# Orbis-Tertius/tiny-ram-halo2

Measured on AMD Instinct MI355X. Metric: Pallas MSM pairs/s @ 2^24 + Fp NTT elems/s @ 2^22; 1/2/4/8 MI355X, higher is better.
Workload: dtype u255 (255-bit modular integers as 9 x 29/30-bit limbs in i32 / i64 lanes)

## Files before the change

tiny-ram-halo2_amd/csrc/msm.hip:

```cpp
#include <stdlib.h>
#include <string.h>

#include "ctx.h"
#include "devmem.h"
#include "curve_q4.h"
#include "hostcombine.h"
#include "hosthelper.h"
#include "hostplan.h"

namespace trh {

namespace {

using hostplan::MAX_C; using hostplan::MAX_C_FIXED; using hostplan::MSM_TILE; using hostplan::SMALL_C; using hostplan::SMALL_MAX_N;
using hostplan::PART_TILE; using hostplan::BIN_THREADS; using hostplan::BIN_PER_MAX; using hostplan::BIN_CAP_MAX; using hostplan::RANGE_BLOCK;
using hostplan::HEAVY_PIECES; using hostplan::SP_LISTS; using hostplan::SP_CNT; using hostplan::SP_PAD; using hostplan::SP_PARTS; using hostplan::SP_MAX_CHUNK;
using hostplan::num_windows;
static_assert(sizeof(XYZZMem) == hostplan::XYZZ_BYTES && sizeof(XYZZzMem) == hostplan::RAW_POINT_BYTES, "point sizes of the plan's scratch layout");
constexpr u32 SIGN_BIT = 0x80000000u;

constexpr int RECODE_THREADS_MAX = 1024;
template <class SF, int C, bool ONE_ROW , bool USE_LDS,
          bool FLAGS >
__global__ void __launch_bounds__(RECODE_THREADS_MAX) msm_recode_kernel(const uint4* __restrict__ scalars, size_t n, int mont, int c_arg, int W,
                                                         u32* __restrict__ digits, u32* __restrict__ bin_counts, int k2, u32 nbins, size_t sstride,
                                                         const uint4* __restrict__ tails ,
                                                         unsigned char* __restrict__ tile_flags, u32 tile_log, u32 tiles) {
    const size_t z = blockIdx.z;
    const u32 rows = ONE_ROW ? 1u : (u32)W;
    scalars += z * sstride * 2; digits += z * (size_t)W * n; bin_counts += z * (size_t)rows * nbins;
    extern __shared__ u32 lhist[];
    const u32 total = rows * nbins;
    if (USE_LDS) {
        for (u32 k = threadIdx.x; k < total; k += blockDim.x) lhist[k] = 0;
        __syncthreads();
    }
    const int c = C ? C : c_arg;
    const u32 mask = (1u << c) - 1u, half = 1u << (c - 1);
    const size_t stride = (size_t)gridDim.x * blockDim.x;
    size_t i = (size_t)blockIdx.x * blockDim.x + threadIdx.x;
    uint4 lo = make_uint4(0, 0, 0, 0), hi = lo;
    if (i < n) {
        const uint4* src = (tails && i == n - 1) ? tails + 2 * z : scalars + 2 * i;
        lo = src[0]; hi = src[1];
        asm volatile("" : "+v"(lo.x), "+v"(lo.y), "+v"(lo.z), "+v"(lo.w), "+v"(hi.x), "+v"(hi.y), "+v"(hi.z), "+v"(hi.w));
    }
    while (i < n) {
        u32 w[8] = {lo.x, lo.y, lo.z, lo.w, hi.x, hi.y, hi.z, hi.w};
        {
            const size_t nx = i + stride < n ? i + stride : i;
            const uint4* src = (tails && nx == n - 1) ? tails + 2 * z : scalars + 2 * nx;
            lo = src[0]; hi = src[1];
        }
        if (mont) fe_store(fe_from_mont(fe_load<SF>(w)), w);
        u32 carry = 0;
        u32* dg = digits + i;
        u32 row = 0;
        size_t slot = i;
        auto emit = [&](u32 raw) {
            raw += carry;
            u32 bucket, sign = 0;
            if (raw > half) { bucket = (1u << c) - raw; carry = 1; sign = SIGN_BIT; }
            else { bucket = raw; carry = 0; }
            *dg = bucket ? (bucket | sign) : 0u;
            if (FLAGS) {
                const unsigned long long nz = __ballot(bucket != 0);
                const u32 lane = threadIdx.x & 63u;
                if (bucket && ((nz & ((1ull << lane) - 1ull)) == 0ull || (slot & (((size_t)1 << tile_log) - 1)) < 64))
                    tile_flags[z * tiles + (slot >> tile_log)] = 1;
                slot += n;
            }
            if (bucket) {
                const u32 bin = (bucket - 1u) >> k2;
                if (USE_LDS) atomicAdd(&lhist[row + bin], 1u);
                else atomicAdd(&bin_counts[(size_t)row + bin], 1u);
            }
            dg += n;
            if (!ONE_ROW) row += nbins;
        };
        if constexpr (C != 0) {
            constexpr int WC = 255 / C + 1;
#pragma unroll
            for (int j = 0; j < WC; ++j) {
                const int b = j * C, k = b >> 5, s = b & 31;
                const u32 a0 = k < 8 ? w[k < 8 ? k : 7] : 0u, a1 = (s + C > 32 && k + 1 < 8) ? w[k + 1 < 8 ? k + 1 : 7] : 0u;
                emit((s ? (a0 >> s) | (a1 << ((32 - s) & 31)) : a0) & mask);
            }
        } else {
            for (int j = 0; j < W; ++j) {
                const u32 raw = w[0] & mask;
#pragma unroll
                for (int k = 0; k < 7; ++k) w[k] = (w[k] >> c) | (w[k + 1] << (32 - c));
                w[7] >>= c;
                emit(raw);
            }
        }
        i += stride;
    }
    if (USE_LDS) {
        __syncthreads();
        for (u32 k = threadIdx.x; k < total; k += blockDim.x) {
            const u32 v = lhist[k];
            if (v) atomicAdd(&bin_counts[k], v);
        }
    }
}

struct ZeroRanges { uint4* p[4]; u32 n16[4]; };
__global__ void __launch_bounds__(256) msm_zero_ranges_kernel(const ZeroRanges z) {
    const uint4 zero = make_uint4(0, 0, 0, 0);
#pragma unroll
    for (int k = 0; k < 4; ++k)
        for (u32 i = blockIdx.x * blockDim.x + threadIdx.x; i < z.n16[k]; i += gridDim.x * blockDim.x) z.p[k][i] = zero;
}

__global__ void __launch_bounds__(1024) msm_offsets_kernel(u32* __restrict__ counts, u32* __restrict__ starts, u32 nb1, u32* __restrict__ oversize, u32 bin_cap,
                                                           u32* __restrict__ totals ) {
    const size_t z = blockIdx.z;
    counts += z * (size_t)gridDim.x * nb1; starts += z * (size_t)gridDim.x * nb1;
    __shared__ u32 part[1024];
    const int j = blockIdx.x, t = threadIdx.x;
    u32* cnt = counts + (size_t)j * nb1;
    u32* st = starts + (size_t)j * nb1;
    const u32 per = (nb1 + 1023u) / 1024u;
    const u32 lo = t * per < nb1 ? t * per : nb1, hi = (lo + per < nb1) ? lo + per : nb1;
    u32 sum = 0, biggest = 0;
    for (u32 b = lo; b < hi; ++b) { const u32 v = cnt[b]; sum += v; biggest = v > biggest ? v : biggest; }
    if (oversize && biggest > bin_cap) atomicMax(oversize + z * gridDim.x + blockIdx.x, biggest);
    part[t] = sum;
    __syncthreads();
    for (int off = 1; off < 1024; off <<= 1) {
        u32 v = (t >= off) ? part[t - off] : 0;
        __syncthreads();
        part[t] += v;
        __syncthreads();
    }
    if (totals && t == 1023) totals[z * gridDim.x + blockIdx.x] = part[1023];
    u32 run = part[t] - sum;
    for (u32 b = lo; b < hi; ++b) {
        u32 cv = cnt[b];
        st[b] = run;
        cnt[b] = run;
        run += cv;
    }
}

constexpr int PART_THREADS = 1024;
__global__ void __launch_bounds__(PART_THREADS) msm_partition_kernel(const u32* __restrict__ digits, u32* __restrict__ bin_cursor,
                                                                     u32* __restrict__ parted, size_t n, int k2, u32 nbins, int idx_bits,
                                                                     const unsigned char* __restrict__ tile_flags ) {
    const size_t z = blockIdx.z;
    if (tile_flags && !tile_flags[z * gridDim.x + blockIdx.x]) return;
    digits += z * (size_t)gridDim.y * n; parted += z * (size_t)gridDim.y * n; bin_cursor += z * (size_t)gridDim.y * nbins;
    extern __shared__ u32 lds[];
    u32* stage = lds;
    u32* cnt = lds + PART_TILE;
    u32* lbase = cnt + nbins;
    u32* gbase = lbase + nbins;
    __shared__ u32 scan[PART_THREADS];
    const int j = blockIdx.y;
    const size_t t0 = (size_t)blockIdx.x * PART_TILE;
    const size_t t1 = t0 + PART_TILE < n ? t0 + PART_TILE : n;
    const u32* dg = digits + (size_t)j * n;
    for (u32 k = threadIdx.x; k < nbins; k += blockDim.x) cnt[k] = 0;
    __syncthreads();
    constexpr int PER = PART_TILE / PART_THREADS;
    u32 mine[PER];
#pragma unroll
    for (int q = 0; q < PER; ++q) {
        const size_t i = t0 + threadIdx.x + (size_t)q * PART_THREADS;
        mine[q] = i < t1 ? dg[i] : 0u;
    }
#pragma unroll
    for (int q = 0; q < PER; ++q) {
        const u32 b = mine[q] & ~SIGN_BIT;
        if (b) atomicAdd(&cnt[(b - 1u) >> k2], 1u);
    }
    __syncthreads();
    {
        const u32 per = (nbins + PART_THREADS - 1) / PART_THREADS;
        const u32 lo = threadIdx.x * per < nbins ? threadIdx.x * per : nbins, hi = lo + per < nbins ? lo + per : nbins;
        u32 sum = 0;
        for (u32 k = lo; k < hi; ++k) sum += cnt[k];
        scan[threadIdx.x] = sum;
        __syncthreads();
        for (int off = 1; off < PART_THREADS; off <<= 1) {
            const u32 v = ((int)threadIdx.x >= off) ? scan[threadIdx.x - off] : 0;
            __syncthreads();
            scan[threadIdx.x] += v;
            __syncthreads();
        }
        u32 run = scan[threadIdx.x] - sum;
        for (u32 k = lo; k < hi; ++k) {
            const u32 v = cnt[k];
            lbase[k] = run;
            gbase[k] = v ? atomicAdd(&bin_cursor[(size_t)j * nbins + k], v) : 0u;
            run += v;
        }
    }
    __syncthreads();
    for (u32 k = threadIdx.x; k < nbins; k += blockDim.x) cnt[k] = 0;
    __syncthreads();
    const u32 low_mask = (1u << k2) - 1u;
#pragma unroll
    for (int q = 0; q < PER; ++q) {
        const u32 e = mine[q];
        const u32 b = e & ~SIGN_BIT;
        if (b) {
            const u32 bm = b - 1u, bin = bm >> k2;
            const u32 r = atomicAdd(&cnt[bin], 1u);
            stage[lbase[bin] + r] = (u32)(t0 + threadIdx.x + (size_t)q * PART_THREADS) | ((bm & low_mask) << idx_bits) | (e & SIGN_BIT);
        }
    }
    __syncthreads();
    u32* out = parted + (size_t)j * n;
    const u32 wave = threadIdx.x >> 6, lane = threadIdx.x & 63u;
    for (u32 bin = wave; bin < nbins; bin += PART_THREADS / 64) {
        const u32 c = cnt[bin], lb = lbase[bin], gb = gbase[bin];
        for (u32 k = lane; k < c; k += 64) out[gb + k] = stage[lb + k];
    }
}

constexpr int BS_CHUNK = 8192;
constexpr int BS_THREADS = 512;

__device__ __forceinline__ u32 bin_of_position(const u32* __restrict__ bin_ends, u32 nbins, u32 pos) {
    u32 lo = 0, hi = nbins;
    while (lo < hi) {
        const u32 mid = (lo + hi) >> 1;
        if (bin_ends[mid] > pos) hi = mid; else lo = mid + 1;
    }
    return lo;
}

template <bool SCATTER>
__global__ void __launch_bounds__(BS_THREADS) msm_bucket_pass_kernel(const u32* __restrict__ parted, const u32* __restrict__ bin_starts,
                                                                     const u32* __restrict__ bin_ends, u32* __restrict__ bucket_cnt ,
                                                                     u32* __restrict__ sorted, size_t n, int k2, u32 nbins, int idx_bits, u32 nbk,
                                                                     const u32* __restrict__ oversize) {
    const size_t z = blockIdx.z;
    {
        const size_t Wz = gridDim.y;
        parted += z * Wz * n; sorted += z * Wz * n; bin_starts += z * Wz * nbins; bin_ends += z * Wz * nbins;
        bucket_cnt += z * Wz * (nbk + 1);
    }
    if (oversize && oversize[z * gridDim.y + blockIdx.y] == 0u) return;
    __shared__ u32 cnt[128], tbase[128], gbase[128];
    __shared__ u32 stage[SCATTER ? BS_CHUNK : 1];
    const int j = blockIdx.y;
    const u32* bs = bin_starts + (size_t)j * nbins;
    const u32* be = bin_ends + (size_t)j * nbins;
    const u32 total = be[nbins - 1];
    const u32 c0 = blockIdx.x * BS_CHUNK;
    if (c0 >= total) return;
    const u32 c1 = c0 + BS_CHUNK < total ? c0 + BS_CHUNK : total;
    const u32 nsub = 1u << k2, low_mask = nsub - 1u, idx_mask = (1u << idx_bits) - 1u;
    const u32* src = parted + (size_t)j * n;
    u32* dst = sorted + (size_t)j * n;
    u32* bc = bucket_cnt + (size_t)j * (nbk + 1);
    const u32 wave = threadIdx.x >> 6, lane = threadIdx.x & 63u;
    for (u32 bin = bin_of_position(be, nbins, c0); bin < nbins; ++bin) {
        const u32 lo = bs[bin] > c0 ? bs[bin] : c0;
        if (lo >= c1) break;
        const u32 hi = be[bin] < c1 ? be[bin] : c1;
        if (hi <= lo) continue;
        if (hi - lo <= 64u) {
            if (threadIdx.x < hi - lo) {
                const u32 e = src[lo + threadIdx.x];
                u32* cell = &bc[(bin << k2) + ((e >> idx_bits) & low_mask) + 1u];
                if (!SCATTER) atomicAdd(cell, 1u);
                else dst[atomicAdd(cell, 1u)] = (e & idx_mask) | (e & SIGN_BIT);
            }
            continue;
        }
        if (threadIdx.x < 128) cnt[threadIdx.x] = 0;
        __syncthreads();
        for (u32 i = lo + threadIdx.x; i < hi; i += blockDim.x) atomicAdd(&cnt[(src[i] >> idx_bits) & low_mask], 1u);
        __syncthreads();
        if (!SCATTER) {
            if (threadIdx.x < nsub && cnt[threadIdx.x]) atomicAdd(&bc[(bin << k2) + threadIdx.x + 1u], cnt[threadIdx.x]);
        } else {
            if (threadIdx.x == 0) {
                u32 r = 0;
                for (u32 k = 0; k < nsub; ++k) { tbase[k] = r; r += cnt[k]; }
            }
            if (threadIdx.x < nsub) {
                const u32 v = cnt[threadIdx.x];
                gbase[threadIdx.x] = v ? atomicAdd(&bc[(bin << k2) + threadIdx.x + 1u], v) : 0u;
            }
            __syncthreads();
            if (threadIdx.x < 128) cnt[threadIdx.x] = 0;
            __syncthreads();
            for (u32 i = lo + threadIdx.x; i < hi; i += blockDim.x) {
                const u32 e = src[i];
                const u32 sub = (e >> idx_bits) & low_mask;
                const u32 r = atomicAdd(&cnt[sub], 1u);
                stage[tbase[sub] + r] = (e & idx_mask) | (e & SIGN_BIT);
            }
            __syncthreads();
            for (u32 sub = wave; sub < nsub; sub += BS_THREADS / 64) {
                const u32 c = cnt[sub], sb = tbase[sub], gb = gbase[sub];
                for (u32 k = lane; k < c; k += 64) dst[gb + k] = stage[sb + k];
            }
        }
        __syncthreads();
    }
}

template <int PER>
__global__ void __launch_bounds__(BIN_THREADS) msm_bin_sort_kernel(const u32* __restrict__ parted, const u32* __restrict__ bin_starts, const u32* __restrict__ bin_ends,
                                                                   u32* __restrict__ sorted, u32* __restrict__ starts, u32* __restrict__ ends, size_t n, int k2, u32 nbins,
                                                                   int idx_bits, u32 nbk, const u32* __restrict__ oversize) {
    if (oversize[(size_t)blockIdx.z * gridDim.y + blockIdx.y] != 0u) return;
    extern __shared__ u32 bstage[];
    __shared__ u32 cnt[128], tbase[128], wave0_total;
    const size_t z = blockIdx.z, Wz = gridDim.y;
    const int j = blockIdx.y;
    const u32 bin = blockIdx.x;
    const size_t wrow = z * Wz + j;
    const u32 lo = bin_starts[wrow * nbins + bin], hi = bin_ends[wrow * nbins + bin];
    const u32 count = hi - lo;
    const u32 nsub = 1u << k2, low_mask = nsub - 1u, idx_mask = (1u << idx_bits) - 1u;
    const u32* src = parted + wrow * n + lo;
    u32* dst = sorted + wrow * n + lo;
    const u32 lane = threadIdx.x & 63u;
    if (threadIdx.x < 128) cnt[threadIdx.x] = 0;
    __syncthreads();
    u32 mine[PER];
#pragma unroll
    for (int q = 0; q < PER; ++q) {
        const u32 i = threadIdx.x + (u32)q * BIN_THREADS;
        mine[q] = (u32)q * BIN_THREADS < count ? src[i < count ? i : 0u] : 0u;
    }
#pragma unroll
    for (int q = 0; q < PER; ++q)
        if (threadIdx.x + (u32)q * BIN_THREADS < count) atomicAdd(&cnt[(mine[q] >> idx_bits) & low_mask], 1u);
    __syncthreads();
    u32 v = 0, x = 0;
    if (threadIdx.x < 128) {
        v = threadIdx.x < nsub ? cnt[threadIdx.x] : 0u;
        x = v;
#pragma unroll
        for (int off = 1; off < 64; off <<= 1) {
            const u32 y = __shfl_up(x, off, 64);
            if ((int)lane >= off) x += y;
        }
        if (threadIdx.x == 63) wave0_total = x;
    }
    __syncthreads();
    if (threadIdx.x < 128) {
        const u32 excl = x - v + (threadIdx.x >= 64 ? wave0_total : 0u);
        tbase[threadIdx.x] = excl;
        cnt[threadIdx.x] = 0;
        if (threadIdx.x < nsub) {
            const size_t b = wrow * (nbk + 1) + ((size_t)bin << k2) + threadIdx.x + 1u;
            starts[b] = lo + excl;
            ends[b] = lo + excl + v;
        }
        if (bin == 0 && threadIdx.x == 0) { starts[wrow * (nbk + 1)] = 0; ends[wrow * (nbk + 1)] = 0; }
    }
    __syncthreads();
#pragma unroll
    for (int q = 0; q < PER; ++q) {
        if (threadIdx.x + (u32)q * BIN_THREADS < count) {
            const u32 e = mine[q];
            const u32 sub = (e >> idx_bits) & low_mask;
            const u32 r = atomicAdd(&cnt[sub], 1u);
            bstage[tbase[sub] + r] = (e & idx_mask) | (e & SIGN_BIT);
        }
    }
    __syncthreads();
#pragma unroll
    for (int q = 0; q < PER; ++q) {
        const u32 i = threadIdx.x + (u32)q * BIN_THREADS;
        if (i < count) mine[q] = bstage[i];
    }
#pragma unroll
    for (int q = 0; q < PER; ++q) {
        const u32 i = threadIdx.x + (u32)q * BIN_THREADS;
        if (i < count) dst[i] = mine[q];
    }
}

__global__ void __launch_bounds__(RANGE_BLOCK) msm_bucket_block_sums_kernel(const u32* __restrict__ bucket_cnt, u32* __restrict__ block_sums, u32 nbk,
                                                                            const u32* __restrict__ oversize) {
    if (oversize && oversize[(size_t)blockIdx.z * gridDim.y + blockIdx.y] == 0u) return;
    __shared__ u32 part[RANGE_BLOCK / 64];
    const size_t z = blockIdx.z, Wz = gridDim.y;
    const u32 nb1 = nbk + 1, b = blockIdx.x * RANGE_BLOCK + threadIdx.x;
    u32 v = b < nb1 ? bucket_cnt[(z * Wz + blockIdx.y) * nb1 + b] : 0u;
#pragma unroll
    for (int off = 32; off > 0; off >>= 1) v += __shfl_down(v, off, 64);
    if ((threadIdx.x & 63) == 0) part[threadIdx.x >> 6] = v;
    __syncthreads();
    if (threadIdx.x == 0) {
        u32 t = 0;
        for (int k = 0; k < RANGE_BLOCK / 64; ++k) t += part[k];
        block_sums[(z * Wz + blockIdx.y) * gridDim.x + blockIdx.x] = t;
    }
}
__global__ void __launch_bounds__(RANGE_BLOCK) msm_bucket_ranges_kernel(u32* __restrict__ bucket_cnt, const u32* __restrict__ block_sums, u32* __restrict__ starts,
                                                                        u32* __restrict__ ends, u32 nbk, const u32* __restrict__ oversize) {
    if (oversize && oversize[(size_t)blockIdx.z * gridDim.y + blockIdx.y] == 0u) return;
    __shared__ u32 part[RANGE_BLOCK];
    __shared__ u32 before;
    const size_t z = blockIdx.z, Wz = gridDim.y;
    const int t = threadIdx.x;
    const u32 nb1 = nbk + 1, b = blockIdx.x * RANGE_BLOCK + t;
    const size_t row = (z * Wz + blockIdx.y) * nb1;
    const u32 c = b < nb1 ? bucket_cnt[row + b] : 0u;
    {
        u32 v = (u32)t < blockIdx.x ? block_sums[(z * Wz + blockIdx.y) * gridDim.x + t] : 0u;
        part[t] = v;
        __syncthreads();
        for (int s = RANGE_BLOCK / 2; s > 0; s >>= 1) {
            if (t < s) part[t] += part[t + s];
            __syncthreads();
        }
        if (t == 0) before = part[0];
        __syncthreads();
    }
    part[t] = c;
    __syncthreads();
    for (int off = 1; off < RANGE_BLOCK; off <<= 1) {
        const u32 v = (t >= off) ? part[t - off] : 0;
        __syncthreads();
        part[t] += v;
        __syncthreads();
    }
    if (b < nb1) {
        const u32 E = before + part[t], S = E - c;
        starts[row + b] = S; ends[row + b] = E; bucket_cnt[row + b] = S;
    }
}

template <class BF>
__device__ __forceinline__ void store_zrec(uint4* q, const Fy<BF>& x, const Fy<BF>& y) {
    q[0] = make_uint4((u32)x.l[0], (u32)x.l[1], (u32)x.l[2], (u32)x.l[3]); q[1] = make_uint4((u32)x.l[4], (u32)x.l[5], (u32)x.l[6], (u32)x.l[7]);
    q[2] = make_uint4((u32)y.l[0], (u32)y.l[1], (u32)y.l[2], (u32)y.l[3]); q[3] = make_uint4((u32)y.l[4], (u32)y.l[5], (u32)y.l[6], (u32)y.l[7]);
    q[4] = make_uint4((u32)-y.l[0], (u32)-y.l[1], (u32)-y.l[2], (u32)-y.l[3]); q[5] = make_uint4((u32)-y.l[4], (u32)-y.l[5], (u32)-y.l[6], (u32)-y.l[7]);
    q[6] = make_uint4((u32)x.l[8], (u32)y.l[8], (u32)-y.l[8], 0u);
    q[7] = make_uint4(0u, 0u, 0u, 0u);
}
template <class BF>
__global__ void __launch_bounds__(256) msm_convert_bases_kernel(const uint4* __restrict__ in, uint4* __restrict__ out, size_t n) {
    size_t i = (size_t)blockIdx.x * blockDim.x + threadIdx.x;
    if (i >= n) return;
    const uint4* p = in + i * 4;
    uint4 a = p[0], b = p[1], c = p[2], d = p[3];
    store_zrec(out + i * (ZREC / 16), fy_from_fe(fe_load<BF>(a.x, a.y, a.z, a.w, b.x, b.y, b.z, b.w)), fy_from_fe(fe_load<BF>(c.x, c.y, c.z, c.w, d.x, d.y, d.z, d.w)));
}

template <class BF>
__global__ void __launch_bounds__(256) msm_accumulate_seg_kernel(const uint4* __restrict__ bases_z, const u32* __restrict__ sorted,
                                                                 const u32* __restrict__ ends,
                                                                 XYZZzMem* __restrict__ first, XYZZzMem* __restrict__ last,
                                                                 XYZZzMem* __restrict__ direct, size_t n, u32 nbk, u32 nseg, u32 seg_len,
                                                                 const u32* __restrict__ lean_gate ) {
    const size_t z = blockIdx.z;
    if (lean_gate && lean_gate[z * gridDim.y + blockIdx.y] != 0u) return;
    {
        const size_t Wz = gridDim.y;
        sorted += z * Wz * n; ends += z * Wz * (nbk + 1);
        first += z * Wz * nseg; last += z * Wz * nseg; direct += z * Wz * (nbk + 1);
    }
    const u32 t = blockIdx.x * blockDim.x + threadIdx.x;
    const int j = blockIdx.y;
    if (t >= nseg) return;
    const u32 nb1 = nbk + 1;
    const u32* en = ends + (size_t)j * nb1;
    const u32 total = en[nbk];
    u32 pos = t * seg_len;
    if (pos >= total) return;
    const u32 stop = pos + seg_len < total ? pos + seg_len : total;
    u32 B;
    {
        u32 lo = 0, hi = nbk;
        while (lo < hi) {
            const u32 mid = (lo + hi) >> 1;
            if (en[mid] > pos) hi = mid; else lo = mid + 1;
        }
        B = lo;
    }
    u32 cur_end = en[B];
    const u32* lst = sorted + (size_t)j * n;
    XYZZzMem* my_first = first + (size_t)j * nseg + t;
    XYZZz<BF> acc = xyzzz_identity<BF>();
    bool is_first = true;
    bool fresh = true;
    struct Slot { u32 e; uint4 a, b, c, d, t; };
    auto issue = [&](Slot& sl, u32 entry) {
        sl.e = entry;
        const uint4* bp = bases_z + (size_t)(entry & ~SIGN_BIT) * (ZREC / 16);
        const uint4* yp = bp + 2 + ((entry >> 31) << 1);
        sl.a = bp[0]; sl.b = bp[1]; sl.c = yp[0]; sl.d = yp[1]; sl.t = bp[6];
    };
    auto unpack = [&](const Slot& sl, AffineZ<BF>& p) {
        p.x.l[0] = (i32)sl.a.x; p.x.l[1] = (i32)sl.a.y; p.x.l[2] = (i32)sl.a.z; p.x.l[3] = (i32)sl.a.w;
        p.x.l[4] = (i32)sl.b.x; p.x.l[5] = (i32)sl.b.y; p.x.l[6] = (i32)sl.b.z; p.x.l[7] = (i32)sl.b.w; p.x.l[8] = (i32)sl.t.x;
        p.y.l[0] = (i32)sl.c.x; p.y.l[1] = (i32)sl.c.y; p.y.l[2] = (i32)sl.c.z; p.y.l[3] = (i32)sl.c.w;
        p.y.l[4] = (i32)sl.d.x; p.y.l[5] = (i32)sl.d.y; p.y.l[6] = (i32)sl.d.z; p.y.l[7] = (i32)sl.d.w; p.y.l[8] = (i32)((sl.e >> 31) ? sl.t.z : sl.t.y);
    };
    const u32 last_pos = stop - 1;
    auto clamp = [&](u32 q) { return q < last_pos ? q : last_pos; };
    Slot s0, s1;
    issue(s0, lst[pos]);
    issue(s1, lst[clamp(pos + 1)]);
    u32 e_ahead = lst[clamp(pos + 2)];
    auto step = [&](Slot& sl) {
        if (pos == cur_end) {
            store_raw(is_first ? my_first : direct + (size_t)j * nb1 + B, acc);
            is_first = false;
            fresh = true;
            int walked = 0;
            do { ++B; cur_end = en[B]; } while (cur_end <= pos && ++walked < 4);
            if (cur_end <= pos) {
                u32 lo = B + 1, hi = nbk;
                while (lo < hi) {
                    const u32 mid = (lo + hi) >> 1;
                    if (en[mid] > pos) hi = mid; else lo = mid + 1;
                }
                B = lo;
// ... 1309 lines not shown
```

Baseline: 1.048 billion.

## Flatten partition write-out and swizzle blocks across XCDs

The partition kernel now remaps its block ids so consecutive work items land on the same XCD (8-way swizzle). The final copy from LDS stage to global output no longer walks bins per wave. Each thread instead takes a flat stage slot, finds its bin from a compact staged word, and writes to the slot position plus a per-bin delta (global base minus local base). This is meant to fix load imbalance from small or uneven bins and to improve L2 locality, at the cost of an extra LDS lookup per element and re-encoding the output word.

Result: no change. 1.055 billion, median of 6 (+0.6%).

```diff
diff --git a/tiny-ram-halo2_amd/csrc/msm.hip b/tiny-ram-halo2_amd/csrc/msm.hip
--- a/tiny-ram-halo2_amd/csrc/msm.hip
+++ b/tiny-ram-halo2_amd/csrc/msm.hip
@@ -146,20 +146,31 @@
 }
 
 constexpr int PART_THREADS = 1024;
+constexpr int PART_LOCAL_BITS = 14;
+constexpr u32 PART_XCDS = 8;
+static_assert(PART_TILE == 1 << PART_LOCAL_BITS, "the staged word keeps the index inside the tile in PART_LOCAL_BITS bits");
+static_assert(PART_LOCAL_BITS + (MAX_C - 1) <= 31 && PART_LOCAL_BITS + (MAX_C_FIXED - 1) <= 31, "staged word: tile index, bucket - 1 < 2^(c - 1), sign");
 __global__ void __launch_bounds__(PART_THREADS) msm_partition_kernel(const u32* __restrict__ digits, u32* __restrict__ bin_cursor,
                                                                      u32* __restrict__ parted, size_t n, int k2, u32 nbins, int idx_bits,
                                                                      const unsigned char* __restrict__ tile_flags ) {
     const size_t z = blockIdx.z;
-    if (tile_flags && !tile_flags[z * gridDim.x + blockIdx.x]) return;
+    u32 tile = blockIdx.x, j = blockIdx.y;
+    {
+        const u32 items = gridDim.x * gridDim.y, per = items / PART_XCDS, id = blockIdx.x + gridDim.x * blockIdx.y;
+        if (id < per * PART_XCDS) {
+            const u32 m = (id % PART_XCDS) * per + id / PART_XCDS;
+            tile = m % gridDim.x; j = m / gridDim.x;
+        }
+    }
+    if (tile_flags && !tile_flags[z * gridDim.x + tile]) return;
     digits += z * (size_t)gridDim.y * n; parted += z * (size_t)gridDim.y * n; bin_cursor += z * (size_t)gridDim.y * nbins;
     extern __shared__ u32 lds[];
     u32* stage = lds;
     u32* cnt = lds + PART_TILE;
     u32* lbase = cnt + nbins;
-    u32* gbase = lbase + nbins;
+    u32* delta = lbase + nbins;
     __shared__ u32 scan[PART_THREADS];
-    const int j = blockIdx.y;
-    const size_t t0 = (size_t)blockIdx.x * PART_TILE;
+    const size_t t0 = (size_t)tile * PART_TILE;
     const size_t t1 = t0 + PART_TILE < n ? t0 + PART_TILE : n;
     const u32* dg = digits + (size_t)j * n;
     for (u32 k = threadIdx.x; k < nbins; k += blockDim.x) cnt[k] = 0;
@@ -193,15 +204,15 @@
         u32 run = scan[threadIdx.x] - sum;
         for (u32 k = lo; k < hi; ++k) {
             const u32 v = cnt[k];
+            const u32 gb = v ? atomicAdd(&bin_cursor[(size_t)j * nbins + k], v) : 0u;
             lbase[k] = run;
-            gbase[k] = v ? atomicAdd(&bin_cursor[(size_t)j * nbins + k], v) : 0u;
+            delta[k] = gb - run;
             run += v;
         }
     }
     __syncthreads();
     for (u32 k = threadIdx.x; k < nbins; k += blockDim.x) cnt[k] = 0;
     __syncthreads();
-    const u32 low_mask = (1u << k2) - 1u;
 #pragma unroll
     for (int q = 0; q < PER; ++q) {
         const u32 e = mine[q];
@@ -209,15 +220,28 @@
         if (b) {
             const u32 bm = b - 1u, bin = bm >> k2;
             const u32 r = atomicAdd(&cnt[bin], 1u);
-            stage[lbase[bin] + r] = (u32)(t0 + threadIdx.x + (size_t)q * PART_THREADS) | ((bm & low_mask) << idx_bits) | (e & SIGN_BIT);
+            stage[lbase[bin] + r] = (threadIdx.x + (u32)q * PART_THREADS) | (bm << PART_LOCAL_BITS) | (e & SIGN_BIT);
         }
     }
     __syncthreads();
     u32* out = parted + (size_t)j * n;
-    const u32 wave = threadIdx.x >> 6, lane = threadIdx.x & 63u;
-    for (u32 bin = wave; bin < nbins; bin += PART_THREADS / 64) {
-        const u32 c = cnt[bin], lb = lbase[bin], gb = gbase[bin];
-        for (u32 k = lane; k < c; k += 64) out[gb + k] = stage[lb + k];
+    const u32 total = scan[PART_THREADS - 1], low_mask = (1u << k2) - 1u, local_mask = (1u << PART_LOCAL_BITS) - 1u;
+#pragma unroll
+    for (int q = 0; q < PER; ++q) {
+        const u32 p = threadIdx.x + (u32)q * PART_THREADS;
+        mine[q] = stage[p < total ? p : 0u];
+    }
+    u32 dst[PER];
+#pragma unroll
+    for (int q = 0; q < PER; ++q) {
+        const u32 p = threadIdx.x + (u32)q * PART_THREADS;
+        dst[q] = delta[p < total ? (mine[q] & ~SIGN_BIT) >> (PART_LOCAL_BITS + k2) : 0u] + p;
+    }
+#pragma unroll
+    for (int q = 0; q < PER; ++q) {
+        const u32 p = threadIdx.x + (u32)q * PART_THREADS;
+        const u32 w = mine[q];
+        if (p < total) out[dst[q]] = ((u32)t0 + (w & local_mask)) | (((w >> PART_LOCAL_BITS) & low_mask) << idx_bits) | (w & SIGN_BIT);
     }
 }
 
```

## Reuse counting-pass ranks and flatten scatter in MSM partition kernel

Applied to the files above, without the earlier changes.

The partition kernel now records each element's rank from the first LDS atomic counting pass, packing two 16-bit ranks per register. This removes the second counter reset and the second round of LDS atomics. The staged word holds the full bucket-minus-one and the tile-local index. The final write-out becomes one flat loop over all staged slots that decodes the bin with bitfield extracts and adds a per-bin global delta, replacing the per-wave-per-bin loop that left lanes idle on small bins. The cost is more live registers, per-slot decode work and a new bit-budget constraint checked by a static_assert.

Result: no change. 1.067 billion before, 1.067 billion after (median of 2 runs) (-0.0%).

```diff
diff --git a/tiny-ram-halo2_amd/csrc/msm.hip b/tiny-ram-halo2_amd/csrc/msm.hip
--- a/tiny-ram-halo2_amd/csrc/msm.hip
+++ b/tiny-ram-halo2_amd/csrc/msm.hip
@@ -146,6 +146,8 @@
 }
 
 constexpr int PART_THREADS = 1024;
+constexpr int PART_TILE_LOG = 14;
+static_assert(PART_TILE == 1 << PART_TILE_LOG && hostplan::MAX_C - 1 + PART_TILE_LOG + 1 <= 32 && hostplan::MAX_C_FIXED <= hostplan::MAX_C, "staged word of msm_partition_kernel");
 __global__ void __launch_bounds__(PART_THREADS) msm_partition_kernel(const u32* __restrict__ digits, u32* __restrict__ bin_cursor,
                                                                      u32* __restrict__ parted, size_t n, int k2, u32 nbins, int idx_bits,
                                                                      const unsigned char* __restrict__ tile_flags ) {
@@ -156,7 +158,7 @@
     u32* stage = lds;
     u32* cnt = lds + PART_TILE;
     u32* lbase = cnt + nbins;
-    u32* gbase = lbase + nbins;
+    u32* gdelta = lbase + nbins;
     __shared__ u32 scan[PART_THREADS];
     const int j = blockIdx.y;
     const size_t t0 = (size_t)blockIdx.x * PART_TILE;
@@ -171,10 +173,15 @@
         const size_t i = t0 + threadIdx.x + (size_t)q * PART_THREADS;
         mine[q] = i < t1 ? dg[i] : 0u;
     }
+    u32 rank2[PER / 2];
 #pragma unroll
     for (int q = 0; q < PER; ++q) {
         const u32 b = mine[q] & ~SIGN_BIT;
-        if (b) atomicAdd(&cnt[(b - 1u) >> k2], 1u);
+        if (!(q & 1)) rank2[q / 2] = 0u;
+        if (b) {
+            const u32 r = atomicAdd(&cnt[(b - 1u) >> k2], 1u);
+            rank2[q / 2] = (q & 1) ? (r << 16) | rank2[q / 2] : r;
+        }
     }
     __syncthreads();
     {
@@ -194,30 +201,29 @@
         for (u32 k = lo; k < hi; ++k) {
             const u32 v = cnt[k];
             lbase[k] = run;
-            gbase[k] = v ? atomicAdd(&bin_cursor[(size_t)j * nbins + k], v) : 0u;
+            gdelta[k] = (v ? atomicAdd(&bin_cursor[(size_t)j * nbins + k], v) : 0u) - run;
             run += v;
         }
     }
     __syncthreads();
-    for (u32 k = threadIdx.x; k < nbins; k += blockDim.x) cnt[k] = 0;
-    __syncthreads();
-    const u32 low_mask = (1u << k2) - 1u;
 #pragma unroll
     for (int q = 0; q < PER; ++q) {
         const u32 e = mine[q];
         const u32 b = e & ~SIGN_BIT;
         if (b) {
-            const u32 bm = b - 1u, bin = bm >> k2;
-            const u32 r = atomicAdd(&cnt[bin], 1u);
-            stage[lbase[bin] + r] = (u32)(t0 + threadIdx.x + (size_t)q * PART_THREADS) | ((bm & low_mask) << idx_bits) | (e & SIGN_BIT);
+            const u32 bm = b - 1u, r = (q & 1) ? rank2[q / 2] >> 16 : rank2[q / 2] & 0xFFFFu;
+            stage[lbase[bm >> k2] + r] = (e & SIGN_BIT) | (bm << PART_TILE_LOG) | (threadIdx.x + q * PART_THREADS);
         }
     }
     __syncthreads();
     u32* out = parted + (size_t)j * n;
-    const u32 wave = threadIdx.x >> 6, lane = threadIdx.x & 63u;
-    for (u32 bin = wave; bin < nbins; bin += PART_THREADS / 64) {
-        const u32 c = cnt[bin], lb = lbase[bin], gb = gbase[bin];
-        for (u32 k = lane; k < c; k += 64) out[gb + k] = stage[lb + k];
+    const u32 total = lbase[nbins - 1u] + cnt[nbins - 1u];
+    const u32 tile_idx = (u32)t0;
+#pragma unroll 4
+    for (u32 sl = threadIdx.x; sl < total; sl += PART_THREADS) {
+        const u32 w = stage[sl];
+        const u32 bin = __builtin_amdgcn_ubfe(w, PART_TILE_LOG + k2, 31 - PART_TILE_LOG - k2), sub = __builtin_amdgcn_ubfe(w, PART_TILE_LOG, k2);
+        out[sl + gdelta[bin]] = (w & (SIGN_BIT | (u32)(PART_TILE - 1))) | ((sub << idx_bits) | tile_idx);
     }
 }
 
```
